# geekieo/collaborative-deep-metric-learning

Hardware: AMD Instinct MI355X
Metric: triplets/sec (higher is better)
Workload: dtype f32 values as 3 exact bf16 planes (hi + mid + lo == the f32 value), 6 bf16-MFMA plane products per f32 product, f32 accumulate

## Files before the change

### collaborative-deep-metric-learning_amd/csrc/optim.hip

```cpp
#include "common.h"
#include <string.h>
#include <type_traits>

namespace cdml {

char *err_buf() {
  static thread_local char buf[512] = {0};
  return buf;
}

int fail(int code, const char *fmt, ...) {
  va_list ap;
  va_start(ap, fmt);
  vsnprintf(err_buf(), 512, fmt, ap);
  va_end(ap);
  return code;
}

namespace {

constexpr int kThreads = 256;
constexpr int kLarsBlocks = 1024;

__device__ __forceinline__ void adam1(float &w, const float g, float &m, float &v, const float omb1,
                                      const float omb2, const float lr_t, const float eps) {
  m = __fmaf_rn(g - m, omb1, m);
  v = __fmaf_rn(__fmaf_rn(g, g, -v), omb2, v);
  w = w - __fdiv_rn(m * lr_t, __fsqrt_rn(v) + eps);
}

__device__ __forceinline__ void lars1(float &w, const float g, float &a, const float slr, const float momentum,
                                      const float wd) {
  a = __fmaf_rn(momentum, a, slr * __fmaf_rn(wd, w, g));
  w = w - a;
}

__device__ __forceinline__ void momentum1(float &w, const float g, float &a, const float lr, const float momentum,
                                          const int nesterov) {
  a = __fmaf_rn(a, momentum, g);
  w = w - (nesterov ? __fmaf_rn(g, lr, a * momentum * lr) : a * lr);
}

__device__ __forceinline__ float adam_lr_t(float &s_lr_t, const float lr_imm, const float *lr_dev, const float b1,
                                           const float b2, const int64_t t_imm, const uint64_t *t_dev) {
  if (threadIdx.x == 0) {
    const double t = (double)t_imm + (t_dev ? (double)(*t_dev) : 0.0);
    const double lr = lr_dev ? (double)(*lr_dev) : (double)lr_imm;
    s_lr_t = (float)(lr * sqrt(1.0 - pow((double)b2, t)) / (1.0 - pow((double)b1, t)));
  }
  __syncthreads();
  return s_lr_t;
}

template <class F>
__device__ __forceinline__ void bias_ride(const int bn, F &&update1) {
  for (int i = blockIdx.x * kThreads + threadIdx.x; i < bn; i += gridDim.x * kThreads) update1(i);
}

__global__ void __launch_bounds__(kThreads)
k_adam(float *__restrict__ w, const float *__restrict__ g, float *__restrict__ m,
       float *__restrict__ v, int64_t n, float lr_imm, const float *__restrict__ lr_dev, float b1,
       float b2, float eps, int64_t t_imm, uint64_t *__restrict__ t_dev, int advance,
       uint32_t *__restrict__ tickets) {
  __shared__ float s_lr_t;
  const float lr_t = adam_lr_t(s_lr_t, lr_imm, lr_dev, b1, b2, t_imm, t_dev);
  const float omb1 = 1.0f - b1, omb2 = 1.0f - b2;
  const int64_t n4 = n >> 2;
  const int64_t stride = (int64_t)gridDim.x * blockDim.x;
  for (int64_t i = (int64_t)blockIdx.x * blockDim.x + threadIdx.x; i < n4; i += stride) {
    float4 w4 = reinterpret_cast<float4 *>(w)[i];
    const float4 g4 = reinterpret_cast<const float4 *>(g)[i];
    float4 m4 = reinterpret_cast<float4 *>(m)[i];
    float4 v4 = reinterpret_cast<float4 *>(v)[i];
#define CDML_ADAM1(c) adam1(w4.c, g4.c, m4.c, v4.c, omb1, omb2, lr_t, eps);
    CDML_ADAM1(x) CDML_ADAM1(y) CDML_ADAM1(z) CDML_ADAM1(w)
#undef CDML_ADAM1
    reinterpret_cast<float4 *>(w)[i] = w4;
    reinterpret_cast<float4 *>(m)[i] = m4;
    reinterpret_cast<float4 *>(v)[i] = v4;
  }
  for (int64_t i = (n4 << 2) + (int64_t)blockIdx.x * blockDim.x + threadIdx.x; i < n; i += stride) {
    float wi = w[i], mi = m[i], vi = v[i];
    adam1(wi, g[i], mi, vi, omb1, omb2, lr_t, eps);
    m[i] = mi;
    v[i] = vi;
    w[i] = wi;
  }
  if (advance && grid_last_block(tickets) && threadIdx.x == 0) *t_dev += 1;
}

constexpr int kAT = 64;
template <int PLANES>
__device__ __forceinline__ void tile_copies(float (&res)[2][2][4], uint32_t (&sT)[64][64 / 2 + 1], __bf16 *__restrict__ wt,
                                            int64_t ldt, __bf16 *__restrict__ wc, int64_t ldc, int64_t plane_t,
                                            int64_t plane_c, int k0, int n0, float h2_scale) {
  using word = std::conditional_t<PLANES == 2, _Float16, __bf16>;
  using word4 = __attribute__((ext_vector_type(4))) word;
  using word2 = __attribute__((ext_vector_type(2))) word;
  const int tr = threadIdx.x >> 4, c4 = (threadIdx.x & 15) * 4;
  if constexpr (PLANES == 2) {
#pragma unroll
    for (int p = 0; p < 2; ++p)
#pragma unroll
      for (int q = 0; q < 2; ++q)
#pragma unroll
        for (int u = 0; u < 4; ++u) res[p][q][u] = __builtin_amdgcn_fmed3f(res[p][q][u] * h2_scale, -65504.f, 65504.f);
  }
#pragma unroll
  for (int pl = 0; pl < PLANES; ++pl) {
    if (pl && wt) __syncthreads();
#pragma unroll
    for (int p = 0; p < 2; ++p) {
      const int r = p * 32 + 2 * tr;
      word4 o[2];
#pragma unroll
      for (int q = 0; q < 2; ++q) {
#pragma unroll
        for (int u = 0; u < 4; ++u) {
          o[q][u] = (word)res[p][q][u];
          if (PLANES > 1) res[p][q][u] -= (float)o[q][u];
        }
        if (wc) *reinterpret_cast<word4 *>(wc + (int64_t)(k0 + r + q) * ldc + pl * plane_c + n0 + c4) = o[q];
      }
#pragma unroll
      for (int u = 0; u < 4; ++u) {
        const word2 pr = {o[0][u], o[1][u]};
        sT[c4 + u][r >> 1] = __builtin_bit_cast(uint32_t, pr);
      }
    }
    if (wt) {
      __syncthreads();
      const int sr = threadIdx.x >> 3, seg = (threadIdx.x & 7) * 4;
#pragma unroll
      for (int q = 0; q < 2; ++q) {
        const int row = q * 32 + sr;
        uint4 o;
        o.x = sT[row][seg]; o.y = sT[row][seg + 1]; o.z = sT[row][seg + 2]; o.w = sT[row][seg + 3];
        *reinterpret_cast<uint4 *>(wt + (int64_t)(n0 + row) * ldt + pl * plane_t + k0 + seg * 2) = o;
      }
    }
  }
}

template <int PLANES, class F>
__device__ __forceinline__ void tile_update(const int N, uint32_t (&sT)[64][64 / 2 + 1], __bf16 *__restrict__ wt, int64_t ldt,
                                            __bf16 *__restrict__ wc, int64_t ldc, int64_t plane_t, int64_t plane_c,
                                            float h2_scale, F &&update4) {
  const int tiles_n = N / kAT;
  const int k0 = (blockIdx.x / tiles_n) * kAT, n0 = (blockIdx.x % tiles_n) * kAT;
  const int tr = threadIdx.x >> 4, c4 = (threadIdx.x & 15) * 4;
  float res[2][2][4];
#pragma unroll
  for (int p = 0; p < 2; ++p) {
    const int r = p * 32 + 2 * tr;
#pragma unroll
    for (int q = 0; q < 2; ++q) {
      const float4 w4 = update4((int64_t)(k0 + r + q) * N + n0 + c4);
      res[p][q][0] = w4.x; res[p][q][1] = w4.y; res[p][q][2] = w4.z; res[p][q][3] = w4.w;
    }
  }
  tile_copies<PLANES>(res, sT, wt, ldt, wc, ldc, plane_t, plane_c, k0, n0, h2_scale);
}

template <int PLANES>
__global__ void __launch_bounds__(kThreads)
k_adam_matrix_bf16(float *__restrict__ w, const float *__restrict__ g, float *__restrict__ m,
                   float *__restrict__ v, int K, int N, float lr_imm, const float *__restrict__ lr_dev,
                   float b1, float b2, float eps, int64_t t_imm, uint64_t *__restrict__ t_dev,
                   __bf16 *__restrict__ wt, int64_t ldt, __bf16 *__restrict__ wc, int64_t ldc,
                   float *__restrict__ bw, const float *__restrict__ bg, float *__restrict__ bm,
                   float *__restrict__ bv, int bn, int advance, uint32_t *__restrict__ tickets,
                   int64_t plane_t, int64_t plane_c, float h2_scale) {
  __shared__ float s_lr_t;
  __shared__ uint32_t sT[kAT][kAT / 2 + 1];
  const float lr_t = adam_lr_t(s_lr_t, lr_imm, lr_dev, b1, b2, t_imm, t_dev);
  const float omb1 = 1.0f - b1, omb2 = 1.0f - b2;
  tile_update<PLANES>(N, sT, wt, ldt, wc, ldc, plane_t, plane_c, h2_scale, [=](const int64_t i) {
    float4 w4 = *reinterpret_cast<float4 *>(w + i);
    const float4 g4 = *reinterpret_cast<const float4 *>(g + i);
    float4 m4 = *reinterpret_cast<float4 *>(m + i);
    float4 v4 = *reinterpret_cast<float4 *>(v + i);
#define CDML_ADAM1(c) adam1(w4.c, g4.c, m4.c, v4.c, omb1, omb2, lr_t, eps);
    CDML_ADAM1(x) CDML_ADAM1(y) CDML_ADAM1(z) CDML_ADAM1(w)
#undef CDML_ADAM1
    *reinterpret_cast<float4 *>(w + i) = w4;
    *reinterpret_cast<float4 *>(m + i) = m4;
    *reinterpret_cast<float4 *>(v + i) = v4;
    return w4;
  });
  if (bw)
    bias_ride(bn, [=](const int i) {
      float wi = bw[i], mi = bm[i], vi = bv[i];
      adam1(wi, bg[i], mi, vi, omb1, omb2, lr_t, eps);
      bm[i] = mi;
      bv[i] = vi;
      bw[i] = wi;
    });
  if (advance && grid_last_block(tickets) && threadIdx.x == 0) *t_dev += 1;
}

__device__ __forceinline__ void block_pair_sum(double (&s)[2][kThreads / kWave], float sw, float sg, float *out) {
  sw = wave_sum(sw);
  sg = wave_sum(sg);
  const int lane = threadIdx.x & (kWave - 1), wave = threadIdx.x >> 6;
  if (lane == 0) { s[0][wave] = sw; s[1][wave] = sg; }
  __syncthreads();
  if (threadIdx.x == 0) {
    double a = 0, b = 0;
    for (int k = 0; k < kThreads / kWave; ++k) { a += s[0][k]; b += s[1][k]; }
    out[0] = (float)a;
    out[1] = (float)b;
  }
}

__device__ __forceinline__ float lars_trust(const float wn, const float gn, const float eeta, const float wd, const float eps) {
  return (wn > 0.f && gn > 0.f) ? eeta * wn / (gn + wd * wn + eps) : 1.0f;
}

template <class F>
__device__ __forceinline__ void lars_segment_norms(double (&s_part)[2][kThreads / kWave], const float *scratch,
                                                   const int b0, const int b1, F &&thread0) {
  const int lane = threadIdx.x & (kWave - 1), wave = threadIdx.x >> 6;
  double a = 0, c = 0;
  for (int k = b0 + threadIdx.x; k < b1; k += kThreads) {
    a += (double)scratch[2 * k];
    c += (double)scratch[2 * k + 1];
  }
#pragma unroll
  for (int o = kWave / 2; o > 0; o >>= 1) {
    a += __shfl_xor(a, o, kWave);
    c += __shfl_xor(c, o, kWave);
  }
  if (lane == 0) { s_part[0][wave] = a; s_part[1][wave] = c; }
  __syncthreads();
  if (threadIdx.x == 0) {
    double wn2 = 0, gn2 = 0;
    for (int k = 0; k < kThreads / kWave; ++k) { wn2 += s_part[0][k]; gn2 += s_part[1][k]; }
    thread0(sqrtf((float)wn2), sqrtf((float)gn2));
  }
  __syncthreads();
}

__global__ void __launch_bounds__(kThreads)
k_lars_norm_partial(const float *__restrict__ w, const float *__restrict__ g, int64_t n,
                    float *__restrict__ scratch) {
  __shared__ double s[2][kThreads / kWave];
  float sw = 0.f, sg = 0.f;
  for (int64_t i = (int64_t)blockIdx.x * blockDim.x + threadIdx.x; i < n;
       i += (int64_t)gridDim.x * blockDim.x) {
    const float a = w[i], b = g[i];
    sw += a * a;
    sg += b * b;
  }
  block_pair_sum(s, sw, sg, scratch + (2 + 2 * blockIdx.x));
}

__global__ void k_lars_norm_final(float *__restrict__ scratch, int blocks) {
  if (threadIdx.x == 0 && blockIdx.x == 0) {
    double a = 0, b = 0;
    for (int k = 0; k < blocks; ++k) { a += scratch[2 + 2 * k]; b += scratch[3 + 2 * k]; }
    scratch[0] = (float)a;
    scratch[1] = (float)b;
  }
}

__global__ void __launch_bounds__(kThreads)
k_lars_apply(float *__restrict__ w, const float *__restrict__ g, float *__restrict__ acc, int64_t n,
             float lr_imm, const float *__restrict__ lr_dev, float momentum, float wd, float eeta,
             float eps, const float *__restrict__ scratch) {
  const float lr = lr_dev ? *lr_dev : lr_imm;
  const float wn = sqrtf(scratch[0]), gn = sqrtf(scratch[1]);
  const float slr = lr * lars_trust(wn, gn, eeta, wd, eps);
  for (int64_t i = (int64_t)blockIdx.x * blockDim.x + threadIdx.x; i < n;
       i += (int64_t)gridDim.x * blockDim.x) {
    float wi = w[i], a = acc[i];
    lars1(wi, g[i], a, slr, momentum, wd);
    acc[i] = a;
    w[i] = wi;
  }
}

constexpr int kMaxSeg = 8;
struct LarsSegs {
  int n_seg;
  int64_t off[kMaxSeg + 1];
  int blk[kMaxSeg + 1];
};

__global__ void __launch_bounds__(kThreads)
k_lars_multi_norms(const float *__restrict__ w, const float *__restrict__ g, LarsSegs S,
                   float *__restrict__ scratch) {
  __shared__ double s[2][kThreads / kWave];
  int seg = 0;
#pragma unroll
  for (int k = 1; k < kMaxSeg; ++k) seg += (k < S.n_seg && (int)blockIdx.x >= S.blk[k]) ? 1 : 0;
  const int nb = S.blk[seg + 1] - S.blk[seg], b = blockIdx.x - S.blk[seg];
  const int64_t lo4 = S.off[seg] >> 2, hi4 = S.off[seg + 1] >> 2;
  float sw = 0.f, sg = 0.f;
  for (int64_t i = lo4 + (int64_t)b * kThreads + threadIdx.x; i < hi4; i += (int64_t)nb * kThreads) {
    const float4 a = reinterpret_cast<const float4 *>(w)[i];
    const float4 c = reinterpret_cast<const float4 *>(g)[i];
    sw += a.x * a.x + a.y * a.y + a.z * a.z + a.w * a.w;
    sg += c.x * c.x + c.y * c.y + c.z * c.z + c.w * c.w;
  }
  block_pair_sum(s, sw, sg, scratch + 2 * blockIdx.x);
}

__global__ void __launch_bounds__(kThreads)
k_lars_multi_apply(float *__restrict__ w, const float *__restrict__ g, float *__restrict__ acc, LarsSegs S,
                   float lr_imm, const float *__restrict__ lr_dev, float momentum, float wd, float eeta,
                   float eps, const float *__restrict__ scratch, float *__restrict__ norms_out,
                   uint64_t *__restrict__ step_dev, uint32_t *__restrict__ tickets) {
  __shared__ double s_part[2][kThreads / kWave];
  __shared__ float s_slr[kMaxSeg];
  const float lr = lr_dev ? *lr_dev : lr_imm;
  for (int seg = 0; seg < S.n_seg; ++seg)
    lars_segment_norms(s_part, scratch, S.blk[seg], S.blk[seg + 1], [=](const float wn, const float gn) {
      s_slr[seg] = lr * lars_trust(wn, gn, eeta, wd, eps);
      if (norms_out && blockIdx.x == 0) { norms_out[2 * seg] = wn; norms_out[2 * seg + 1] = gn; }
    });
  const int64_t n4 = S.off[S.n_seg] >> 2;
  for (int64_t i = (int64_t)blockIdx.x * kThreads + threadIdx.x; i < n4; i += (int64_t)gridDim.x * kThreads) {
    int seg = 0;
#pragma unroll
    for (int k = 1; k < kMaxSeg; ++k) seg += (k < S.n_seg && 4 * i >= S.off[k]) ? 1 : 0;
    const float slr = s_slr[seg];
    float4 w4 = reinterpret_cast<float4 *>(w)[i];
    const float4 g4 = reinterpret_cast<const float4 *>(g)[i];
    float4 a4 = reinterpret_cast<float4 *>(acc)[i];
#define CDML_LARS1(c) lars1(w4.c, g4.c, a4.c, slr, momentum, wd);
    CDML_LARS1(x) CDML_LARS1(y) CDML_LARS1(z) CDML_LARS1(w)
#undef CDML_LARS1
    reinterpret_cast<float4 *>(acc)[i] = a4;
    reinterpret_cast<float4 *>(w)[i] = w4;
  }
  if (step_dev && grid_last_block(tickets) && threadIdx.x == 0) *step_dev += 1;
}

struct MatRule {
  float lr_imm; const float *lr_dev;
  float momentum, wd, eeta, eps;
  int nesterov;
  const float *scratch;
  int blk_w0, blk_w1, blk_b0, blk_b1;
  float *norms_w, *norms_b;
  float h2_scale;
};

template <int RULE>
__device__ __forceinline__ void rule1(float &w, const float g, float &a, const float rate, const float momentum, const float wd,
                                      const int nesterov) {
  if (RULE == 1) lars1(w, g, a, rate, momentum, wd);
  else momentum1(w, g, a, rate, momentum, nesterov);
}

template <int PLANES, int RULE>
__global__ void __launch_bounds__(kThreads)
k_rule_matrix(float *__restrict__ w, const float *__restrict__ g, float *__restrict__ acc, int K, int N, MatRule R,
              __bf16 *__restrict__ wt, int64_t ldt, __bf16 *__restrict__ wc, int64_t ldc, float *__restrict__ bw,
              const float *__restrict__ bg, float *__restrict__ bacc, int bn, uint64_t *__restrict__ step_dev,
              uint32_t *__restrict__ tickets, int64_t plane_t, int64_t plane_c) {
  __shared__ uint32_t sT[kAT][kAT / 2 + 1];
  __shared__ double s_part[2][kThreads / kWave];
  __shared__ float s_slr[2];
  const float lr = R.lr_dev ? *R.lr_dev : R.lr_imm;
  const float momentum = R.momentum, wd = R.wd, eeta = R.eeta, eps = R.eps, h2_scale = R.h2_scale;
  const int nesterov = R.nesterov;
  if (RULE == 1) {
    for (int v = 0; v < 2; ++v) {
      const int b0 = v ? R.blk_b0 : R.blk_w0, b1 = v ? R.blk_b1 : R.blk_w1;
      float *const no = v ? R.norms_b : R.norms_w;
      lars_segment_norms(s_part, R.scratch, b0, b1, [=](const float wn, const float gn) {
        const float trust = lars_trust(wn, gn, eeta, wd, eps);
        s_slr[v] = (b1 > b0) ? lr * trust : lr;
        if (no && blockIdx.x == 0 && b1 > b0) { no[0] = wn; no[1] = gn; }
      });
    }
  }
  const float slr_w = RULE == 1 ? s_slr[0] : lr, slr_b = RULE == 1 ? s_slr[1] : lr;
  tile_update<PLANES>(N, sT, wt, ldt, wc, ldc, plane_t, plane_c, h2_scale, [=](const int64_t i) {
    float4 w4 = *reinterpret_cast<float4 *>(w + i);
    const float4 g4 = *reinterpret_cast<const float4 *>(g + i);
    float4 a4 = *reinterpret_cast<float4 *>(acc + i);
#define CDML_RULE1(c) rule1<RULE>(w4.c, g4.c, a4.c, slr_w, momentum, wd, nesterov);
    CDML_RULE1(x) CDML_RULE1(y) CDML_RULE1(z) CDML_RULE1(w)
#undef CDML_RULE1
    *reinterpret_cast<float4 *>(w + i) = w4;
    *reinterpret_cast<float4 *>(acc + i) = a4;
    return w4;
  });
  if (bw)
    bias_ride(bn, [=](const int i) {
      float wi = bw[i], ai = bacc[i];
      rule1<RULE>(wi, bg[i], ai, slr_b, momentum, wd, nesterov);
      bacc[i] = ai;
      bw[i] = wi;
    });
  if (step_dev && grid_last_block(tickets) && threadIdx.x == 0) *step_dev += 1;
}

__global__ void __launch_bounds__(kThreads)
k_prep_partial(const float *__restrict__ w, const float *__restrict__ g, int64_t n, float l2_scale,
               float *__restrict__ scratch) {
  __shared__ double s[2][kThreads / kWave];
  float sw = 0.f, sg = 0.f;
  for (int64_t i = (int64_t)blockIdx.x * blockDim.x + threadIdx.x; i < n;
       i += (int64_t)gridDim.x * blockDim.x) {
    const float a = w[i], b = g[i] + l2_scale * a;
    sw += a * a;
    sg += b * b;
  }
  block_pair_sum(s, sw, sg, scratch + (2 + 2 * blockIdx.x));
}

__global__ void __launch_bounds__(kThreads)
k_prep_apply(float *__restrict__ g, const float *__restrict__ w, int64_t n, float l2_scale, float clip,
             const float *__restrict__ scratch, float *__restrict__ norms_out) {
  const float gn = sqrtf(scratch[1]);
  const float scale = (clip > 0.f) ? clip / fmaxf(gn, clip) : 1.0f;
  if (norms_out && blockIdx.x == 0 && threadIdx.x == 0) { norms_out[0] = gn; norms_out[1] = scratch[0]; }
  for (int64_t i = (int64_t)blockIdx.x * blockDim.x + threadIdx.x; i < n;
       i += (int64_t)gridDim.x * blockDim.x)
    g[i] = (g[i] + l2_scale * w[i]) * scale;
}

__global__ void __launch_bounds__(kThreads)
k_momentum(float *__restrict__ w, const float *__restrict__ g, float *__restrict__ acc, int64_t n,
           float lr_imm, const float *__restrict__ lr_dev, float momentum, int nesterov) {
  const float lr = lr_dev ? *lr_dev : lr_imm;
  for (int64_t i = (int64_t)blockIdx.x * blockDim.x + threadIdx.x; i < n;
       i += (int64_t)gridDim.x * blockDim.x) {
    float wi = w[i], a = acc[i];
    momentum1(wi, g[i], a, lr, momentum, nesterov);
    acc[i] = a;
    w[i] = wi;
  }
}

int grid_elems(int64_t n, int per_thread) {
  int64_t b = (n / per_thread + kThreads - 1) / kThreads;
  if (b > kNumCU * 8) b = kNumCU * 8;
  return (int)(b < 1 ? 1 : b);
}

}
}

using namespace cdml;

extern "C" int cdml_version(void) { return 3000; }
extern "C" const char *cdml_last_error(void) { return err_buf(); }

extern "C" int cdml_adam_step(float *w, const float *g, float *m, float *v, int64_t n, float lr,
                              const float *lr_dev, float beta1, float beta2, float eps, int64_t t,
                              uint64_t *t_dev, int advance_step, uint32_t *tickets,
                              cdml_stream_t stream) {
  CDML_REQUIRE(w && g && m && v && n > 0, CDML_E_BADARG, "adam_step: bad argument");
  CDML_REQUIRE(!advance_step || (t_dev && tickets), CDML_E_BADARG,
               "adam_step: advance_step needs the device step counter and the ticket words");
  CDML_REQUIRE(t >= (t_dev ? 0 : 1), CDML_E_BADARG, "adam_step: step t is 1-based");
  CDML_REQUIRE(aligned16(w) && aligned16(g) && aligned16(m) && aligned16(v), CDML_E_ALIGN,
               "adam_step: buffers must be 16-B aligned");
  hipLaunchKernelGGL(k_adam, dim3(grid_elems(n, 4)), dim3(kThreads), 0, (hipStream_t)stream, w, g, m,
                     v, n, lr, lr_dev, beta1, beta2, eps, t, t_dev, advance_step, tickets);
  return check_launch("adam_step");
}

template <class... P, class... A>
static void launch_matrix(int planes, void (*k1)(P...), void (*k2)(P...), void (*k3)(P...), int K, int N, cdml_stream_t stream,
                          A... args) {
  hipLaunchKernelGGL(planes == 2 ? k2 : planes == 3 ? k3 : k1, dim3((K / kAT) * (N / kAT)), dim3(kThreads), 0,
                     (hipStream_t)stream, args...);
}

static int check_copies(const char *who, int K, int N, const uint16_t *wt, int64_t ldt, int64_t &plane_t, const uint16_t *wc,
                        int64_t ldc, int64_t &plane_c, int planes) {
  CDML_REQUIRE(planes == 1 || planes == 2 || planes == 3, CDML_E_BADARG, "%s: planes must be 1 (bf16 copies), 2 (fp16 hi | lo) or 3 (hi | mid | lo)", who);
  CDML_REQUIRE(K > 0 && N > 0 && K % kAT == 0 && N % kAT == 0, CDML_E_UNSUPPORTED,
               "%s: K and N must be multiples of 64, got K=%d N=%d", who, K, N);
  CDML_REQUIRE((!wt || (aligned16(wt) && (ldt & 7) == 0 && ldt >= K)) && (!wc || (aligned16(wc) && (ldc & 3) == 0 && ldc >= N)),
               CDML_E_ALIGN, "%s: 16-B aligned copies, ldt a multiple of 8 (>= K), ldc of 4 (>= N)", who);
  if (planes >= 2)
    CDML_REQUIRE((!wt || (!(plane_t & 7) && plane_t >= K && ldt >= (planes - 1) * plane_t + K)) &&
                     (!wc || (!(plane_c & 3) && plane_c >= N && ldc >= (planes - 1) * plane_c + N)),
                 CDML_E_ALIGN, "%s: plane strides (W^T: multiple of 8, >= K; W: multiple of 4, >= N) and leading dimensions "
                 ">= (planes - 1) planes + the matrix width", who);
  else
    plane_t = plane_c = 0;
  return CDML_OK;
}

static int adam_matrix_impl(float *w, const float *g, float *m, float *v, int K, int N, float lr,
                            const float *lr_dev, float beta1, float beta2, float eps, int64_t t,
                            uint64_t *t_dev, uint16_t *wt_bf16, int64_t ldt, uint16_t *wc_bf16,
                            int64_t ldc, float *bias_w, const float *bias_g, float *bias_m,
                            float *bias_v, int bias_n, int advance_step, uint32_t *tickets,
                            int planes, int64_t plane_t, int64_t plane_c, cdml_stream_t stream, float h2_scale = 0.f) {
  CDML_REQUIRE(w && g && m && v && K > 0 && N > 0, CDML_E_BADARG, "adam_matrix_bf16: bad argument");
  CDML_REQUIRE(!bias_w || (bias_g && bias_m && bias_v && bias_n > 0), CDML_E_BADARG,
               "adam_matrix_bf16: the bias vector needs its gradient and both moments");
  CDML_REQUIRE(!advance_step || (t_dev && tickets), CDML_E_BADARG,
               "adam_matrix_bf16: advance_step needs the device step counter and the ticket words");
  CDML_REQUIRE(K % kAT == 0 && N % kAT == 0, CDML_E_UNSUPPORTED,
               "adam_matrix_bf16: K and N must be multiples of 64, got K=%d N=%d", K, N);
  CDML_REQUIRE(t >= (t_dev ? 0 : 1), CDML_E_BADARG, "adam_matrix_bf16: step t is 1-based");
  CDML_REQUIRE(aligned16(w) && aligned16(g) && aligned16(m) && aligned16(v), CDML_E_ALIGN,
               "adam_matrix_bf16: buffers must be 16-B aligned");
  if (int rc = check_copies("adam_matrix_bf16", K, N, wt_bf16, ldt, plane_t, wc_bf16, ldc, plane_c, planes)) return rc;
  CDML_REQUIRE(planes != 2 || h2_scale > 0.f, CDML_E_ALIGN, "adam_matrix_h2: fp16 planes go with a positive scale");
  launch_matrix(planes, k_adam_matrix_bf16<1>, k_adam_matrix_bf16<2>, k_adam_matrix_bf16<3>, K, N, stream, w, g, m, v, K, N, lr,
                lr_dev, beta1, beta2, eps, t, t_dev, reinterpret_cast<__bf16 *>(wt_bf16), ldt, reinterpret_cast<__bf16 *>(wc_bf16),
                ldc, bias_w, bias_g, bias_m, bias_v, bias_w ? bias_n : 0, advance_step, tickets, plane_t, plane_c,
                planes == 2 ? h2_scale : 0.f);
  return check_launch("adam_matrix_bf16");
}

extern "C" int cdml_adam_matrix_bf16(float *w, const float *g, float *m, float *v, int K, int N, float lr,
                                     const float *lr_dev, float beta1, float beta2, float eps, int64_t t,
                                     uint64_t *t_dev, uint16_t *wt_bf16, int64_t ldt, uint16_t *wc_bf16,
                                     int64_t ldc, float *bias_w, const float *bias_g, float *bias_m,
                                     float *bias_v, int bias_n, int advance_step, uint32_t *tickets,
                                     cdml_stream_t stream) {
  return adam_matrix_impl(w, g, m, v, K, N, lr, lr_dev, beta1, beta2, eps, t, t_dev, wt_bf16, ldt, wc_bf16, ldc, bias_w,
                          bias_g, bias_m, bias_v, bias_n, advance_step, tickets, 1, 0, 0, stream);
}

extern "C" int cdml_adam_matrix_planes(float *w, const float *g, float *m, float *v, int K, int N, float lr,
                                       const float *lr_dev, float beta1, float beta2, float eps, int64_t t,
                                       uint64_t *t_dev, uint16_t *wt_planes, int64_t ldt, int64_t plane_t,
                                       uint16_t *wc_planes, int64_t ldc, int64_t plane_c, float *bias_w,
                                       const float *bias_g, float *bias_m, float *bias_v, int bias_n,
                                       int advance_step, uint32_t *tickets, cdml_stream_t stream) {
  return adam_matrix_impl(w, g, m, v, K, N, lr, lr_dev, beta1, beta2, eps, t, t_dev, wt_planes, ldt, wc_planes, ldc, bias_w,
                          bias_g, bias_m, bias_v, bias_n, advance_step, tickets, 3, plane_t, plane_c, stream);
}

extern "C" int cdml_adam_matrix_h2(float *w, const float *g, float *m, float *v, int K, int N, float lr,
                                   const float *lr_dev, float beta1, float beta2, float eps, int64_t t,
                                   uint64_t *t_dev, uint16_t *wt_planes, int64_t ldt, int64_t plane_t,
                                   uint16_t *wc_planes, int64_t ldc, int64_t plane_c, float scale, float *bias_w,
                                   const float *bias_g, float *bias_m, float *bias_v, int bias_n,
                                   int advance_step, uint32_t *tickets, cdml_stream_t stream) {
  return adam_matrix_impl(w, g, m, v, K, N, lr, lr_dev, beta1, beta2, eps, t, t_dev, wt_planes, ldt, wc_planes, ldc, bias_w,
                          bias_g, bias_m, bias_v, bias_n, advance_step, tickets, 2, plane_t, plane_c, stream, scale);
}

extern "C" size_t cdml_lars_scratch_floats(void) { return 2 + 2 * (size_t)kLarsBlocks; }

extern "C" int cdml_lars_step(float *w, const float *g, float *acc, int64_t n, float lr,
                              const float *lr_dev, float momentum, float weight_decay, float eeta,
                              float eps, float *scratch, cdml_stream_t stream) {
  CDML_REQUIRE(w && g && acc && scratch && n > 0, CDML_E_BADARG, "lars_step: bad argument");
  int blocks = grid_elems(n, 8);
  if (blocks > kLarsBlocks) blocks = kLarsBlocks;
  hipStream_t s = (hipStream_t)stream;
  hipLaunchKernelGGL(k_lars_norm_partial, dim3(blocks), dim3(kThreads), 0, s, w, g, n, scratch);
  hipLaunchKernelGGL(k_lars_norm_final, dim3(1), dim3(64), 0, s, scratch, blocks);
  hipLaunchKernelGGL(k_lars_apply, dim3(grid_elems(n, 4)), dim3(kThreads), 0, s, w, g, acc, n, lr,
                     lr_dev, momentum, weight_decay, eeta, eps, scratch);
  return check_launch("lars_step");
}

static int lars_layout(const int64_t *seg_offsets, const int64_t *seg_sizes, int n_seg, LarsSegs &S) {
  CDML_REQUIRE(seg_offsets && seg_sizes, CDML_E_BADARG, "lars: segment arrays required");
  CDML_REQUIRE(n_seg >= 1 && n_seg <= kMaxSeg, CDML_E_UNSUPPORTED, "lars: 1..%d segments, got %d", kMaxSeg, n_seg);
  S.n_seg = n_seg;
  int64_t total = 0;
  for (int k = 0; k < n_seg; ++k) {
    CDML_REQUIRE(seg_sizes[k] > 0 && (seg_sizes[k] & 3) == 0 && seg_offsets[k] == total, CDML_E_BADARG,
                 "lars: segments must tile the buffer contiguously in multiples of 4 floats (segment %d)", k);
    S.off[k] = total;
    total += seg_sizes[k];
  }
  S.off[n_seg] = total;
  const int budget = kLarsBlocks - n_seg;
  int nb = 0;
  for (int k = 0; k < n_seg; ++k) {
    S.blk[k] = nb;
    int64_t want = (seg_sizes[k] / 4 + kThreads * 8 - 1) / (kThreads * 8);
    const int64_t share = 1 + (int64_t)((double)budget * (double)seg_sizes[k] / (double)total);
    if (want > share) want = share;
    nb += (int)(want < 1 ? 1 : want);
  }
  S.blk[n_seg] = nb;
  for (int k = n_seg + 1; k <= kMaxSeg; ++k) { S.off[k] = total; S.blk[k] = nb; }
  return CDML_OK;
}

extern "C" size_t cdml_lars_multi_scratch_floats(void) { return 2 * (size_t)kLarsBlocks; }

extern "C" int cdml_lars_multi(float *w, const float *g, float *acc, const int64_t *seg_offsets,
                               const int64_t *seg_sizes, int n_seg, float lr, const float *lr_dev,
                               float momentum, float weight_decay, float eeta, float eps, float *scratch,
                               float *norms_out, uint64_t *step_dev_advance, uint32_t *tickets,
                               cdml_stream_t stream) {
  CDML_REQUIRE(w && g && acc && scratch && seg_offsets && seg_sizes, CDML_E_BADARG, "lars_multi: bad argument");
  CDML_REQUIRE(!step_dev_advance || tickets, CDML_E_BADARG, "lars_multi: advancing the step counter needs the ticket words");
  CDML_REQUIRE(aligned16(w) && aligned16(g) && aligned16(acc), CDML_E_ALIGN, "lars_multi: buffers must be 16-B aligned");
  LarsSegs S;
  if (int rc = lars_layout(seg_offsets, seg_sizes, n_seg, S)) return rc;
  hipStream_t s = (hipStream_t)stream;
  hipLaunchKernelGGL(k_lars_multi_norms, dim3(S.blk[n_seg]), dim3(kThreads), 0, s, w, g, S, scratch);
  hipLaunchKernelGGL(k_lars_multi_apply, dim3(grid_elems(S.off[n_seg], 4)), dim3(kThreads), 0, s, w, g, acc, S, lr, lr_dev,
                     momentum, weight_decay, eeta, eps, scratch, norms_out, step_dev_advance, tickets);
  return check_launch("lars_multi");
}

extern "C" int cdml_lars_multi_norms(const float *w, const float *g, const int64_t *seg_offsets, const int64_t *seg_sizes,
                                     int n_seg, float *scratch, cdml_stream_t stream) {
  CDML_REQUIRE(w && g && scratch, CDML_E_BADARG, "lars_multi_norms: bad argument");
  CDML_REQUIRE(aligned16(w) && aligned16(g), CDML_E_ALIGN, "lars_multi_norms: buffers must be 16-B aligned");
  LarsSegs S;
  if (int rc = lars_layout(seg_offsets, seg_sizes, n_seg, S)) return rc;
  hipLaunchKernelGGL(k_lars_multi_norms, dim3(S.blk[n_seg]), dim3(kThreads), 0, (hipStream_t)stream, w, g, S, scratch);
  return check_launch("lars_multi_norms");
}

static int lars_matrix_impl(float h2_scale, float *w, const float *g, float *acc, const int64_t *seg_offsets, const int64_t *seg_sizes,
                            int n_seg, int seg_matrix, int seg_bias, int K, int N, float lr, const float *lr_dev,
                            float momentum, float weight_decay, float eeta, float eps, const float *scratch,
                            float *norms_out, uint16_t *wt, int64_t ldt, int64_t plane_t, uint16_t *wc, int64_t ldc,
                            int64_t plane_c, int planes, uint64_t *step_dev_advance, uint32_t *tickets,
                            cdml_stream_t stream) {
  CDML_REQUIRE((planes == 2) == (h2_scale > 0.f), CDML_E_BADARG, "lars_matrix: fp16 planes (planes = 2) go with a positive scale");
  CDML_REQUIRE(w && g && acc && scratch, CDML_E_BADARG, "lars_matrix: bad argument");
  CDML_REQUIRE(!step_dev_advance || tickets, CDML_E_BADARG, "lars_matrix: advancing the step counter needs the ticket words");
  CDML_REQUIRE(aligned16(w) && aligned16(g) && aligned16(acc), CDML_E_ALIGN, "lars_matrix: buffers must be 16-B aligned");
  LarsSegs S;
  if (int rc = lars_layout(seg_offsets, seg_sizes, n_seg, S)) return rc;
  CDML_REQUIRE(seg_matrix >= 0 && seg_matrix < n_seg && seg_bias < n_seg && seg_bias != seg_matrix, CDML_E_BADARG,
               "lars_matrix: segment indices out of range");
  CDML_REQUIRE(seg_sizes[seg_matrix] == (int64_t)K * N, CDML_E_BADARG, "lars_matrix: segment %d holds %lld floats, not %d x %d",
               seg_matrix, (long long)seg_sizes[seg_matrix], K, N);
  if (int rc = check_copies("lars_matrix", K, N, wt, ldt, plane_t, wc, ldc, plane_c, planes)) return rc;
  MatRule R{};
  R.lr_imm = lr; R.lr_dev = lr_dev; R.momentum = momentum; R.wd = weight_decay; R.eeta = eeta; R.eps = eps;
  R.scratch = scratch; R.h2_scale = h2_scale;
  R.blk_w0 = S.blk[seg_matrix]; R.blk_w1 = S.blk[seg_matrix + 1];
  R.norms_w = norms_out ? norms_out + 2 * seg_matrix : nullptr;
  float *bw = nullptr, *bacc = nullptr;
  const float *bg = nullptr;
  int bn = 0;
  if (seg_bias >= 0) {
    R.blk_b0 = S.blk[seg_bias]; R.blk_b1 = S.blk[seg_bias + 1];
    R.norms_b = norms_out ? norms_out + 2 * seg_bias : nullptr;
    bw = w + S.off[seg_bias]; bg = g + S.off[seg_bias]; bacc = acc + S.off[seg_bias];
    bn = (int)seg_sizes[seg_bias];
  }
  const int64_t o = S.off[seg_matrix];
  launch_matrix(planes, k_rule_matrix<1, 1>, k_rule_matrix<2, 1>, k_rule_matrix<3, 1>, K, N, stream, w + o, g + o, acc + o, K, N, R,
                reinterpret_cast<__bf16 *>(wt), ldt, reinterpret_cast<__bf16 *>(wc), ldc, bw, bg, bacc, bn, step_dev_advance,
                tickets, plane_t, plane_c);
  return check_launch("lars_matrix");
}

extern "C" int cdml_lars_matrix(float *w, const float *g, float *acc, const int64_t *seg_offsets, const int64_t *seg_sizes,
                                int n_seg, int seg_matrix, int seg_bias, int K, int N, float lr, const float *lr_dev,
                                float momentum, float weight_decay, float eeta, float eps, const float *scratch,
                                float *norms_out, uint16_t *wt, int64_t ldt, int64_t plane_t, uint16_t *wc, int64_t ldc,
                                int64_t plane_c, int planes, uint64_t *step_dev_advance, uint32_t *tickets,
                                cdml_stream_t stream) {
  CDML_REQUIRE(planes != 2, CDML_E_BADARG, "lars_matrix: fp16 planes take a scale: cdml_lars_matrix_h2");
  return lars_matrix_impl(0.f, w, g, acc, seg_offsets, seg_sizes, n_seg, seg_matrix, seg_bias, K, N, lr, lr_dev, momentum, weight_decay,
                          eeta, eps, scratch, norms_out, wt, ldt, plane_t, wc, ldc, plane_c, planes, step_dev_advance, tickets, stream);
}

extern "C" int cdml_lars_matrix_h2(float *w, const float *g, float *acc, const int64_t *seg_offsets, const int64_t *seg_sizes,
                                   int n_seg, int seg_matrix, int seg_bias, int K, int N, float lr, const float *lr_dev,
                                   float momentum, float weight_decay, float eeta, float eps, const float *scratch,
                                   float *norms_out, uint16_t *wt, int64_t ldt, int64_t plane_t, uint16_t *wc, int64_t ldc,
                                   int64_t plane_c, float scale, uint64_t *step_dev_advance, uint32_t *tickets,
                                   cdml_stream_t stream) {
  return lars_matrix_impl(scale, w, g, acc, seg_offsets, seg_sizes, n_seg, seg_matrix, seg_bias, K, N, lr, lr_dev, momentum, weight_decay,
                          eeta, eps, scratch, norms_out, wt, ldt, plane_t, wc, ldc, plane_c, 2, step_dev_advance, tickets, stream);
}

static int momentum_matrix_impl(float h2_scale, float *w, const float *g, float *acc, int K, int N, float lr, const float *lr_dev,
                                float momentum, int use_nesterov, uint16_t *wt, int64_t ldt, int64_t plane_t,
                                uint16_t *wc, int64_t ldc, int64_t plane_c, int planes, float *bias_w,
                                const float *bias_g, float *bias_acc, int bias_n, uint64_t *step_dev_advance,
                                uint32_t *tickets, cdml_stream_t stream) {
  CDML_REQUIRE((planes == 2) == (h2_scale > 0.f), CDML_E_BADARG, "momentum_matrix: fp16 planes (planes = 2) go with a positive scale");
  CDML_REQUIRE(w && g && acc, CDML_E_BADARG, "momentum_matrix: bad argument");
  CDML_REQUIRE(!bias_w || (bias_g && bias_acc && bias_n > 0), CDML_E_BADARG,
               "momentum_matrix: the bias vector needs its gradient and accumulator");
  CDML_REQUIRE(!step_dev_advance || tickets, CDML_E_BADARG, "momentum_matrix: advancing the step counter needs the ticket words");
  CDML_REQUIRE(aligned16(w) && aligned16(g) && aligned16(acc), CDML_E_ALIGN, "momentum_matrix: buffers must be 16-B aligned");
  if (int rc = check_copies("momentum_matrix", K, N, wt, ldt, plane_t, wc, ldc, plane_c, planes)) return rc;
  MatRule R{};
  R.lr_imm = lr; R.lr_dev = lr_dev; R.momentum = momentum; R.nesterov = use_nesterov; R.h2_scale = h2_scale;
  launch_matrix(planes, k_rule_matrix<1, 2>, k_rule_matrix<2, 2>, k_rule_matrix<3, 2>, K, N, stream, w, g, acc, K, N, R,
                reinterpret_cast<__bf16 *>(wt), ldt, reinterpret_cast<__bf16 *>(wc), ldc, bias_w, bias_g, bias_acc,
                bias_w ? bias_n : 0, step_dev_advance, tickets, plane_t, plane_c);
  return check_launch("momentum_matrix");
}

extern "C" int cdml_momentum_matrix(float *w, const float *g, float *acc, int K, int N, float lr, const float *lr_dev,
                                    float momentum, int use_nesterov, uint16_t *wt, int64_t ldt, int64_t plane_t,
                                    uint16_t *wc, int64_t ldc, int64_t plane_c, int planes, float *bias_w,
                                    const float *bias_g, float *bias_acc, int bias_n, uint64_t *step_dev_advance,
                                    uint32_t *tickets, cdml_stream_t stream) {
  CDML_REQUIRE(planes != 2, CDML_E_BADARG, "momentum_matrix: fp16 planes take a scale: cdml_momentum_matrix_h2");
  return momentum_matrix_impl(0.f, w, g, acc, K, N, lr, lr_dev, momentum, use_nesterov, wt, ldt, plane_t, wc, ldc, plane_c, planes, bias_w,
                              bias_g, bias_acc, bias_n, step_dev_advance, tickets, stream);
}

extern "C" int cdml_momentum_matrix_h2(float *w, const float *g, float *acc, int K, int N, float lr, const float *lr_dev,
                                       float momentum, int use_nesterov, uint16_t *wt, int64_t ldt, int64_t plane_t,
                                       uint16_t *wc, int64_t ldc, int64_t plane_c, float scale, float *bias_w,
                                       const float *bias_g, float *bias_acc, int bias_n, uint64_t *step_dev_advance,
                                       uint32_t *tickets, cdml_stream_t stream) {
  return momentum_matrix_impl(scale, w, g, acc, K, N, lr, lr_dev, momentum, use_nesterov, wt, ldt, plane_t, wc, ldc, plane_c, 2, bias_w,
                              bias_g, bias_acc, bias_n, step_dev_advance, tickets, stream);
}

extern "C" int cdml_grad_prepare(float *g, const float *w, int64_t n, float l2_scale, float clip_norm,
                                 float *scratch, float *norms_out, cdml_stream_t stream) {
  CDML_REQUIRE(g && w && scratch && n > 0, CDML_E_BADARG, "grad_prepare: bad argument");
  int blocks = grid_elems(n, 8);
  if (blocks > kLarsBlocks) blocks = kLarsBlocks;
  hipStream_t s = (hipStream_t)stream;
  hipLaunchKernelGGL(k_prep_partial, dim3(blocks), dim3(kThreads), 0, s, w, g, n, l2_scale, scratch);
  hipLaunchKernelGGL(k_lars_norm_final, dim3(1), dim3(64), 0, s, scratch, blocks);
  hipLaunchKernelGGL(k_prep_apply, dim3(grid_elems(n, 4)), dim3(kThreads), 0, s, g, w, n, l2_scale, clip_norm,
                     scratch, norms_out);
  return check_launch("grad_prepare");
}

extern "C" int cdml_momentum_step(float *w, const float *g, float *acc, int64_t n, float lr,
                                  const float *lr_dev, float momentum, int use_nesterov,
                                  cdml_stream_t stream) {
  CDML_REQUIRE(w && g && acc && n > 0, CDML_E_BADARG, "momentum_step: bad argument");
  hipLaunchKernelGGL(k_momentum, dim3(grid_elems(n, 4)), dim3(kThreads), 0, (hipStream_t)stream, w, g, acc, n, lr,
                     lr_dev, momentum, use_nesterov);
  return check_launch("momentum_step");
}
```

Before: 3.109 million.

## Prefetch optimizer tile inputs early and give each plane its own LDS buffer

The matrix optimizer kernels now issue all global loads for the tile (w, g, m, v or acc) at kernel entry, before the lr/LARS norm computation, so memory latency can overlap the scalar setup. The LDS transpose buffer gets one slot per precision plane, which removes the per-plane __syncthreads and does all transposed writes after a single barrier. The launch bounds also gain a minimum of 4 blocks per CU. In exchange the kernels use more LDS and more registers to hold the prefetched float4s, and the occupancy hint may force register spills.

```diff
diff --git a/collaborative-deep-metric-learning_amd/csrc/optim.hip b/collaborative-deep-metric-learning_amd/csrc/optim.hip
--- a/collaborative-deep-metric-learning_amd/csrc/optim.hip
+++ b/collaborative-deep-metric-learning_amd/csrc/optim.hip
@@ -91,7 +91,10 @@
 
 constexpr int kAT = 64;
 template <int PLANES>
-__device__ __forceinline__ void tile_copies(float (&res)[2][2][4], uint32_t (&sT)[64][64 / 2 + 1], __bf16 *__restrict__ wt,
+using TileLds = uint32_t[PLANES][kAT][kAT / 2 + 1];
+
+template <int PLANES>
+__device__ __forceinline__ void tile_copies(float (&res)[2][2][4], TileLds<PLANES> &sT, __bf16 *__restrict__ wt,
                                             int64_t ldt, __bf16 *__restrict__ wc, int64_t ldc, int64_t plane_t,
                                             int64_t plane_c, int k0, int n0, float h2_scale) {
   using word = std::conditional_t<PLANES == 2, _Float16, __bf16>;
@@ -108,7 +111,6 @@
   }
 #pragma unroll
   for (int pl = 0; pl < PLANES; ++pl) {
-    if (pl && wt) __syncthreads();
 #pragma unroll
     for (int p = 0; p < 2; ++p) {
       const int r = p * 32 + 2 * tr;
@@ -125,37 +127,52 @@
 #pragma unroll
       for (int u = 0; u < 4; ++u) {
         const word2 pr = {o[0][u], o[1][u]};
-        sT[c4 + u][r >> 1] = __builtin_bit_cast(uint32_t, pr);
+        if (wt) sT[pl][c4 + u][r >> 1] = __builtin_bit_cast(uint32_t, pr);
       }
     }
-    if (wt) {
-      __syncthreads();
-      const int sr = threadIdx.x >> 3, seg = (threadIdx.x & 7) * 4;
-#pragma unroll
-      for (int q = 0; q < 2; ++q) {
-        const int row = q * 32 + sr;
-        uint4 o;
-        o.x = sT[row][seg]; o.y = sT[row][seg + 1]; o.z = sT[row][seg + 2]; o.w = sT[row][seg + 3];
-        *reinterpret_cast<uint4 *>(wt + (int64_t)(n0 + row) * ldt + pl * plane_t + k0 + seg * 2) = o;
-      }
+  }
+  if (!wt) return;
+  __syncthreads();
+  const int sr = threadIdx.x >> 3, seg = (threadIdx.x & 7) * 4;
+#pragma unroll
+  for (int pl = 0; pl < PLANES; ++pl) {
+#pragma unroll
+    for (int q = 0; q < 2; ++q) {
+      const int row = q * 32 + sr;
+      uint4 o;
+      o.x = sT[pl][row][seg]; o.y = sT[pl][row][seg + 1]; o.z = sT[pl][row][seg + 2]; o.w = sT[pl][row][seg + 3];
+      *reinterpret_cast<uint4 *>(wt + (int64_t)(n0 + row) * ldt + pl * plane_t + k0 + seg * 2) = o;
     }
   }
 }
 
-template <int PLANES, class F>
-__device__ __forceinline__ void tile_update(const int N, uint32_t (&sT)[64][64 / 2 + 1], __bf16 *__restrict__ wt, int64_t ldt,
-                                            __bf16 *__restrict__ wc, int64_t ldc, int64_t plane_t, int64_t plane_c,
-                                            float h2_scale, F &&update4) {
+__device__ __forceinline__ int64_t tile_elem(const int N, const int p, const int q) {
   const int tiles_n = N / kAT;
   const int k0 = (blockIdx.x / tiles_n) * kAT, n0 = (blockIdx.x % tiles_n) * kAT;
   const int tr = threadIdx.x >> 4, c4 = (threadIdx.x & 15) * 4;
+  return (int64_t)(k0 + p * 32 + 2 * tr + q) * N + n0 + c4;
+}
+
+template <class In, class L>
+__device__ __forceinline__ void tile_load(const int N, In (&in)[2][2], L &&load4) {
+#pragma unroll
+  for (int p = 0; p < 2; ++p)
+#pragma unroll
+    for (int q = 0; q < 2; ++q) in[p][q] = load4(tile_elem(N, p, q));
+}
+
+template <int PLANES, class In, class F>
+__device__ __forceinline__ void tile_update(const int N, TileLds<PLANES> &sT, __bf16 *__restrict__ wt, int64_t ldt,
+                                            __bf16 *__restrict__ wc, int64_t ldc, int64_t plane_t, int64_t plane_c,
+                                            float h2_scale, In (&in)[2][2], F &&update4) {
+  const int tiles_n = N / kAT;
+  const int k0 = (blockIdx.x / tiles_n) * kAT, n0 = (blockIdx.x % tiles_n) * kAT;
   float res[2][2][4];
 #pragma unroll
   for (int p = 0; p < 2; ++p) {
-    const int r = p * 32 + 2 * tr;
 #pragma unroll
     for (int q = 0; q < 2; ++q) {
-      const float4 w4 = update4((int64_t)(k0 + r + q) * N + n0 + c4);
+      const float4 w4 = update4(tile_elem(N, p, q), in[p][q]);
       res[p][q][0] = w4.x; res[p][q][1] = w4.y; res[p][q][2] = w4.z; res[p][q][3] = w4.w;
     }
   }
@@ -163,7 +180,7 @@
 }
 
 template <int PLANES>
-__global__ void __launch_bounds__(kThreads)
+__global__ void __launch_bounds__(kThreads, 4)
 k_adam_matrix_bf16(float *__restrict__ w, const float *__restrict__ g, float *__restrict__ m,
                    float *__restrict__ v, int K, int N, float lr_imm, const float *__restrict__ lr_dev,
                    float b1, float b2, float eps, int64_t t_imm, uint64_t *__restrict__ t_dev,
@@ -172,14 +189,17 @@
                    float *__restrict__ bv, int bn, int advance, uint32_t *__restrict__ tickets,
                    int64_t plane_t, int64_t plane_c, float h2_scale) {
   __shared__ float s_lr_t;
-  __shared__ uint32_t sT[kAT][kAT / 2 + 1];
+  __shared__ TileLds<PLANES> sT;
+  struct In { float4 w, g, m, v; } in[2][2];
+  tile_load(N, in, [=](const int64_t i) {
+    return In{*reinterpret_cast<const float4 *>(w + i), *reinterpret_cast<const float4 *>(g + i),
+              *reinterpret_cast<const float4 *>(m + i), *reinterpret_cast<const float4 *>(v + i)};
+  });
   const float lr_t = adam_lr_t(s_lr_t, lr_imm, lr_dev, b1, b2, t_imm, t_dev);
   const float omb1 = 1.0f - b1, omb2 = 1.0f - b2;
-  tile_update<PLANES>(N, sT, wt, ldt, wc, ldc, plane_t, plane_c, h2_scale, [=](const int64_t i) {
-    float4 w4 = *reinterpret_cast<float4 *>(w + i);
-    const float4 g4 = *reinterpret_cast<const float4 *>(g + i);
-    float4 m4 = *reinterpret_cast<float4 *>(m + i);
-    float4 v4 = *reinterpret_cast<float4 *>(v + i);
+  tile_update<PLANES>(N, sT, wt, ldt, wc, ldc, plane_t, plane_c, h2_scale, in, [=](const int64_t i, const In &x) {
+    float4 w4 = x.w, m4 = x.m, v4 = x.v;
+    const float4 g4 = x.g;
 #define CDML_ADAM1(c) adam1(w4.c, g4.c, m4.c, v4.c, omb1, omb2, lr_t, eps);
     CDML_ADAM1(x) CDML_ADAM1(y) CDML_ADAM1(z) CDML_ADAM1(w)
 #undef CDML_ADAM1
@@ -360,9 +380,14 @@
               __bf16 *__restrict__ wt, int64_t ldt, __bf16 *__restrict__ wc, int64_t ldc, float *__restrict__ bw,
               const float *__restrict__ bg, float *__restrict__ bacc, int bn, uint64_t *__restrict__ step_dev,
               uint32_t *__restrict__ tickets, int64_t plane_t, int64_t plane_c) {
-  __shared__ uint32_t sT[kAT][kAT / 2 + 1];
+  __shared__ TileLds<PLANES> sT;
   __shared__ double s_part[2][kThreads / kWave];
   __shared__ float s_slr[2];
+  struct In { float4 w, g, a; } in[2][2];
+  tile_load(N, in, [=](const int64_t i) {
+    return In{*reinterpret_cast<const float4 *>(w + i), *reinterpret_cast<const float4 *>(g + i),
+              *reinterpret_cast<const float4 *>(acc + i)};
+  });
   const float lr = R.lr_dev ? *R.lr_dev : R.lr_imm;
   const float momentum = R.momentum, wd = R.wd, eeta = R.eeta, eps = R.eps, h2_scale = R.h2_scale;
   const int nesterov = R.nesterov;
@@ -378,10 +403,9 @@
     }
   }
   const float slr_w = RULE == 1 ? s_slr[0] : lr, slr_b = RULE == 1 ? s_slr[1] : lr;
-  tile_update<PLANES>(N, sT, wt, ldt, wc, ldc, plane_t, plane_c, h2_scale, [=](const int64_t i) {
-    float4 w4 = *reinterpret_cast<float4 *>(w + i);
-    const float4 g4 = *reinterpret_cast<const float4 *>(g + i);
-    float4 a4 = *reinterpret_cast<float4 *>(acc + i);
+  tile_update<PLANES>(N, sT, wt, ldt, wc, ldc, plane_t, plane_c, h2_scale, in, [=](const int64_t i, const In &x) {
+    float4 w4 = x.w, a4 = x.a;
+    const float4 g4 = x.g;
 #define CDML_RULE1(c) rule1<RULE>(w4.c, g4.c, a4.c, slr_w, momentum, wd, nesterov);
     CDML_RULE1(x) CDML_RULE1(y) CDML_RULE1(z) CDML_RULE1(w)
 #undef CDML_RULE1
```

New measurement: 3.109 million. Within noise of the previous version (-0.0%).
